# kaiwenShen/Do-You-Really-Need-to-Pay-2-20-Hedge-Fund-Strategy-Replication-via-Machine-Learning

Hardware: AMD Instinct MI355X
Metric: seq/sec/node MTSS-WGAN-GP train (24x32 windows) at 1/2/4/8 GPUs; W-dist parity (higher is better)
Workload: dtype fp32; 1 GPU; global_batch=262144, batch_per_gpu=262144, seq_len=24, features=32, parallelism=dp1

## Files before the change

do-you-really-need-to-pay-2-20-hedge-fund-strategy-replication-via-machine-learning_amd/csrc/bindings.cpp:

```cpp
#include <torch/extension.h>
#include <torch/library.h>
#include <ATen/hip/impl/HIPGuardImplMasqueradingAsCUDA.h>
#include <ATen/hip/impl/HIPStreamMasqueradingAsCUDA.h>

#include "kernels.h"
#include "poison.h"

#include <atomic>
#include <cmath>
#include <cstdlib>
#include <cstring>

std::atomic<bool>& hfrep::poison_flag() {
  static std::atomic<bool> f{[] {
    const char* e = getenv("HFREP_POISON");
    return e && e[0] == '1';
  }()};
  return f;
}

namespace {

using at::Tensor;
using c10::optional;
// ... 210 lines not shown
                                         (int)act, cur_stream(zx));
  TORCH_CHECK(ok, "lstm_fwd: hidden size ", H, " not instantiated (supported: 100, 64, 32)");
  return {hs, gates, cs};
}

Tensor lstm_bwd(Tensor dH, Tensor gates, Tensor cs, Tensor U, int64_t act) {
  CHECK_GPU(dH); CHECK_GPU(gates); CHECK_GPU(cs); same_dt(dH, gates); same_dt(dH, cs);
  const int B = gates.size(0), Tn = gates.size(1), H = gates.size(2) / 4;
  TORCH_CHECK(dH.sizes() == cs.sizes() && cs.size(2) == H, "lstm_bwd: shapes");
  check_lstm_U(U, H);
  GUARD(dH);
  Tensor dZ = out_empty_like(gates);
  const bool ok = hfrep::launch_lstm_bwd(dt_of(dH), dH.data_ptr(), gates.data_ptr(), cs.data_ptr(),
                                         U.data_ptr<float>(), dZ.data_ptr(), B, Tn, H, (int)act, cur_stream(dH));
  TORCH_CHECK(ok, "lstm_bwd: hidden size ", H, " not instantiated");
  return dZ;
}

std::tuple<Tensor, Tensor, Tensor> lstm_tfwd(Tensor dzx, Tensor gates, Tensor cs, Tensor U, int64_t act) {
  CHECK_GPU(dzx); CHECK_GPU(gates); CHECK_GPU(cs); same_dt(dzx, gates); same_dt(dzx, cs);
  TORCH_CHECK(dzx.sizes() == gates.sizes(), "lstm_tfwd: shapes");
  const int B = gates.size(0), Tn = gates.size(1), H = gates.size(2) / 4;
  check_lstm_U(U, H);
  GUARD(dzx);
  Tensor hds = out_empty({B, Tn, H}, dzx.options());
  Tensor zds = out_empty_like(gates);
  Tensor cds = out_empty({B, Tn, H}, dzx.options());
  const bool ok = hfrep::launch_lstm_tfwd(dt_of(dzx), dzx.data_ptr(), gates.data_ptr(), cs.data_ptr(),
                                          U.data_ptr<float>(), hds.data_ptr(), zds.data_ptr(), cds.data_ptr(), B, Tn,
                                          H, (int)act, cur_stream(dzx));
  TORCH_CHECK(ok, "lstm_tfwd: hidden size ", H, " not instantiated");
  return {hds, zds, cds};
}

std::tuple<Tensor, Tensor> lstm_tbwd(optional<Tensor> dH, Tensor dHd, Tensor gates, Tensor cs, Tensor zds, Tensor cds,
                                     Tensor U, int64_t act) {
  CHECK_GPU(dHd); CHECK_GPU(gates); CHECK_GPU(cs); CHECK_GPU(zds); CHECK_GPU(cds);
  same_dt(dHd, gates); same_dt(dHd, zds); same_dt(dHd, cds);
  if (dH.has_value()) { CHECK_GPU(*dH); same_dt(*dH, dHd); }
  const int B = gates.size(0), Tn = gates.size(1), H = gates.size(2) / 4;
  check_lstm_U(U, H);
  GUARD(dHd);
  Tensor dZ = out_empty_like(gates), dZd = out_empty_like(gates);
  const bool ok = hfrep::launch_lstm_tbwd(dt_of(dHd), ptr_or_null(dH), dHd.data_ptr(), gates.data_ptr(),
                                          cs.data_ptr(), zds.data_ptr(), cds.data_ptr(), U.data_ptr<float>(),
                                          dZ.data_ptr(), dZd.data_ptr(), B, Tn, H, (int)act, cur_stream(dHd));
  TORCH_CHECK(ok, "lstm_tbwd: hidden size ", H, " not instantiated");
  return {dZ, dZd};
}

bool lstmf_supported(int64_t H, int64_t K, int64_t act) { return hfrep::lstmf_supported((int)H, (int)K, (int)act); }
bool narrowf_supported(int64_t K, int64_t N) { return hfrep::narrowf_supported((int)K, (int)N); }
int64_t set_lstmf_fwd_impl(int64_t v) { return hfrep::set_lstmf_fwd_impl((int)v); }
int64_t set_lstmf_bwd_impl(int64_t v) { return hfrep::set_lstmf_bwd_impl((int)v); }

std::tuple<Tensor, Tensor> lstmf_fwd(Tensor x, Tensor W, optional<Tensor> b, Tensor U, int64_t act, bool save) {
  CHECK_F32(x); CHECK_F32(W);
  TORCH_CHECK(x.dim() == 3, "x must be (B, T, K)");
  const int B = x.size(0), Tn = x.size(1), K = x.size(2), H = U.size(0);
  check_lstm_U(U, H);
  TORCH_CHECK(W.size(0) == K && W.size(1) == 4 * H, "W must be (K, 4H)");
  if (b.has_value()) { CHECK_F32(*b); TORCH_CHECK(b->numel() == 4 * H, "bias size"); }
  TORCH_CHECK(hfrep::lstmf_supported(H, K, (int)act), "lstmf_fwd: unsupported H/K/act");
  GUARD(x);
  Tensor hs = out_empty({B, Tn, H}, x.options());
  Tensor tape = at::empty({save ? (int64_t)hfrep::lstmf_tape_elems(B, Tn) : 0}, x.options());
  const bool ok = hfrep::launch_lstmf_fwd(x.data_ptr<float>(), W.data_ptr<float>(),
                                          b.has_value() ? b->data_ptr<float>() : nullptr, U.data_ptr<float>(),
                                          hs.data_ptr<float>(), save ? tape.data_ptr<float>() : nullptr, B, Tn, K, H,
                                          (int)act, cur_stream(x));
  TORCH_CHECK(ok, "lstmf_fwd: launch failed");
  return {hs, tape};
}

std::tuple<Tensor, Tensor> lstmf_tfwd(Tensor xd, Tensor W, Tensor U, Tensor tape, int64_t act) {
  CHECK_F32(xd); CHECK_F32(W); CHECK_F32(tape);
  TORCH_CHECK(xd.dim() == 3, "xd must be (B, T, K)");
  const int B = xd.size(0), Tn = xd.size(1), K = xd.size(2), H = U.size(0);
  check_lstm_U(U, H);
  TORCH_CHECK(W.size(0) == K && W.size(1) == 4 * H, "W must be (K, 4H)");
  TORCH_CHECK(tape.numel() == (int64_t)hfrep::lstmf_tape_elems(B, Tn), "lstmf_tfwd: tape size");
  TORCH_CHECK(hfrep::lstmf_supported(H, K, (int)act), "lstmf_tfwd: unsupported H/K/act");
  GUARD(xd);
  Tensor hds = out_empty({B, Tn, H}, xd.options());
  Tensor ttape = at::empty_like(tape);
  const bool ok = hfrep::launch_lstmf_tfwd(xd.data_ptr<float>(), W.data_ptr<float>(), U.data_ptr<float>(),
                                           tape.data_ptr<float>(), hds.data_ptr<float>(), ttape.data_ptr<float>(), B, Tn,
                                           K, H, (int)act, cur_stream(xd));
  TORCH_CHECK(ok, "lstmf_tfwd: launch failed");
  return {hds, ttape};
}

static void check_head(const optional<Tensor>& d, const optional<Tensor>& w, const Tensor& like, int64_t B, int64_t n) {
  if (d.has_value()) {
    CHECK_F32(*d);
    TORCH_CHECK(d->numel() == B && d->device() == like.device(), "head adjoint factor: B fp32 values");
  }
  if (w.has_value()) {
    CHECK_F32(*w);
    TORCH_CHECK(w->numel() == n && w->device() == like.device(), "head weight: Tn H fp32 values");
  }
}

bool lstmf_ahd_supported() { return hfrep::lstmf_ahd_supported(); }

Tensor lstmf_bwd(optional<Tensor> dH, Tensor tape, Tensor U, int64_t act, int64_t B, int64_t Tn, optional<Tensor> hd,
// ... 629 lines not shown
  return (int64_t)reinterpret_cast<intptr_t>(hfrep::p2p_ipc_open(h, (int)device));
}

void p2p_close(int64_t ptr) { hfrep::p2p_ipc_close(reinterpret_cast<void*>((intptr_t)ptr)); }

void p2p_allreduce_(Tensor x, Tensor buf, std::vector<int64_t> peers, int64_t rank, int64_t cap, double scale,
                    double timeout_s) {
  CHECK_F32(x);
  TORCH_CHECK(buf.is_cuda() && buf.scalar_type() == at::kByte && buf.device() == x.device(),
              "p2p_allreduce_: buf must be this device's p2p_buffer");
  const int world = (int)peers.size();
  TORCH_CHECK(world >= 1 && world <= hfrep::kP2PMaxRanks && rank >= 0 && rank < world, "p2p_allreduce_: 1 <= world <= 8");
  TORCH_CHECK(x.numel() <= cap && buf.numel() >= (int64_t)hfrep::p2p_buffer_bytes(cap), "p2p_allreduce_: x exceeds cap");
  TORCH_CHECK(peers[rank] == (int64_t)reinterpret_cast<intptr_t>(buf.data_ptr()), "p2p_allreduce_: peers[rank] must be buf");
  hfrep::P2PPeers pp{};
  for (int r = 0; r < world; ++r) pp.base[r] = reinterpret_cast<char*>((intptr_t)peers[r]);
  TORCH_CHECK(timeout_s > 0, "p2p_allreduce_: timeout_s must be positive");
  GUARD(x);
  static thread_local int s_dev = -1;
  static thread_local double s_sec = -1;
  static thread_local uint64_t s_ticks = 0;
  if (s_dev != x.get_device() || s_sec != timeout_s) {
    s_ticks = hfrep::p2p_timeout_ticks(timeout_s, x.get_device());
    s_dev = x.get_device();
    s_sec = timeout_s;
  }
  hfrep::launch_p2p_allreduce(x.data_ptr<float>(), x.numel(), pp, (int)rank, world, cap, (float)scale, s_ticks,
                              cur_stream(x));
}

int64_t p2p_error(Tensor buf) {
  TORCH_CHECK(buf.is_cuda() && buf.scalar_type() == at::kByte, "p2p_error: a p2p_buffer tensor");
  GUARD(buf);
  return hfrep::p2p_read_error(buf.data_ptr());
}

}

TORCH_LIBRARY(hfrep, m) {
  m.def("linear(Tensor x, Tensor W, Tensor? b, int act, Tensor(a!)? out=None) -> Tensor");
  m.def("linear_dgrad(Tensor dz, Tensor W) -> Tensor");
  m.def("linear_wgrad_(Tensor x, Tensor dz, Tensor(a!) gW, Tensor(b!)? gb, int shiftT=0) -> ()");
  m.def("lstm_wgrad_(Tensor x, Tensor hs, Tensor dZ, Tensor(a!) gW, Tensor(b!) gU, Tensor(c!)? gb, Tensor? xd=None, Tensor? hds=None, Tensor? dZd=None, int impl=0) -> ()");
  m.def("act_fwd(Tensor x, int act) -> Tensor");
  m.def("act_bwd(Tensor dy, Tensor y, int act) -> Tensor");
  m.def("act_tangent_bwd(Tensor dyd, Tensor y, Tensor zd, int act) -> Tensor");
  m.def("lstm_fwd(Tensor zx, Tensor U, int act, bool save) -> (Tensor, Tensor, Tensor)");
  m.def("lstm_bwd(Tensor dH, Tensor gates, Tensor cs, Tensor U, int act) -> Tensor");
  m.def("lstm_tfwd(Tensor dzx, Tensor gates, Tensor cs, Tensor U, int act) -> (Tensor, Tensor, Tensor)");
  m.def("lstm_tbwd(Tensor? dH, Tensor dHd, Tensor gates, Tensor cs, Tensor zds, Tensor cds, Tensor U, int act) -> (Tensor, Tensor)");
  m.def("lstmf_supported(int H, int K, int act) -> bool", &lstmf_supported);
  m.def("narrowf_supported(int K, int N) -> bool", &narrowf_supported);
  m.def("set_lstmf_fwd_impl(int v) -> int", &set_lstmf_fwd_impl);
  m.def("set_lstmf_bwd_impl(int v) -> int", &set_lstmf_bwd_impl);
  m.def("lstmf_fwd(Tensor x, Tensor W, Tensor? b, Tensor U, int act, bool save) -> (Tensor, Tensor)");
  m.def("linear_head_cs(Tensor x, Tensor W, Tensor? b, int split, float wa, float wb, Tensor(a!) gW, Tensor(b!)? gb) -> Tensor");
  m.def("linear_head_cs_supported(int K) -> bool", &linear_head_cs_supported);
  m.def("lstmf_bwd(Tensor? dH, Tensor tape, Tensor U, int act, int B, int T, Tensor? hd=None, Tensor? hw=None, "
        "Tensor(a!)? ah_out=None) -> Tensor");
  m.def("lstmf_ahd_supported() -> bool", &lstmf_ahd_supported);
  m.def("lstmf_tbwd1(Tensor? dH, Tensor aH, Tensor tape, Tensor ttape, Tensor U, int act, int B, int T, Tensor? hd=None, "
        "Tensor? hw=None) -> Tensor");
  m.def("lstmf_tbwd(Tensor? dH, Tensor? dHd, Tensor tape, Tensor ttape, Tensor U, int act, int B, int T, Tensor? hd=None, "
        "Tensor? hdd=None, Tensor? hw=None) -> (Tensor, Tensor)");
  m.def("lstmf_tfwd(Tensor xd, Tensor W, Tensor U, Tensor tape, int act) -> (Tensor, Tensor)");
  m.def("lstmf_dgrad(Tensor dz, Tensor W, int impl=0) -> Tensor");
  m.def("lstm2_fwd(Tensor x, Tensor W, Tensor? b, Tensor U, int act, bool save) -> (Tensor, Tensor)");
  m.def("lstm2_bwd(Tensor? dH, Tensor tape, Tensor U, int act, Tensor? W=None, bool need_dz=True, Tensor? head_d=None, "
        "Tensor? head_w=None) -> (Tensor, Tensor)");
  m.def("lstm2_tfwd(Tensor xd, Tensor W, Tensor U, Tensor tape, int act) -> (Tensor, Tensor)");
  m.def("lstm2_tbwd(Tensor? dH, Tensor? dHd, Tensor tape, Tensor ttape, Tensor U, int act, Tensor? W=None, "
        "Tensor? head_d=None, Tensor? head_dd=None, Tensor? head_w=None) -> (Tensor, Tensor, Tensor, Tensor)");
  m.def("set_debug_poison(bool on) -> bool", &set_debug_poison);
  m.def("layernorm_fwd(Tensor x, Tensor gamma, Tensor beta, float eps, bool save=True, float pre_lrelu=-1.0) -> "
        "(Tensor, Tensor, Tensor)");
  m.def("layernorm_bwd_(Tensor dy, Tensor xhat, Tensor rstd, Tensor gamma, Tensor(a!)? ggamma, Tensor(b!)? gbeta) -> Tensor");
  m.def("layernorm_tfwd(Tensor xd, Tensor xhat, Tensor rstd, Tensor gamma) -> Tensor");
  m.def("layernorm_tbwd_(Tensor? dy, Tensor dyd, Tensor xd, Tensor xhat, Tensor rstd, Tensor gamma, "
        "Tensor(a!) ggamma, Tensor(b!) gbeta, bool need_dx) -> (Tensor, Tensor)");
  m.def("gp_coef(Tensor g, float weight) -> (Tensor, Tensor)");
  m.def("gp_coef_pack(Tensor g, float weight, Tensor w) -> (Tensor, Tensor)");
  m.def("gp_pack(Tensor pen, float weight, Tensor w) -> Tensor");
  m.def("gan_loss(Tensor p, int split, float la, float lb, int kind) -> (Tensor, Tensor)");
  m.def("im2col_causal(Tensor x, int k, int dil) -> Tensor");
  m.def("col2im_causal(Tensor dcols, int k, int dil, int C) -> Tensor");
  m.def("interpolate(Tensor real, Tensor fake, Tensor alpha) -> Tensor");
  m.def("philox_fill_(Tensor(a!) out, int seed, Tensor(b!) ctr, int dist) -> ()");
  m.def("sample_windows(Tensor data, int batch, int seed, Tensor(a!) ctr, ScalarType out_dtype, Tensor(b!)? dst=None) -> Tensor");
  m.def("ae_fit_supported(int A, int k, int batch) -> bool", &ae_fit_supported);
  m.def("ae_fit(Tensor[] Xt, Tensor[] Xv, Tensor[] order, Tensor(a!)[] We, Tensor(b!)[] Wd, Tensor(c!)[] mWe, "
        "Tensor(d!)[] vWe, Tensor(e!)[] mWd, Tensor(f!)[] vWd, Tensor(g!)[] step, Tensor(h!)[] m_cache, int[] patience, "
        "float lr, float b1, float b2, float eps, int batch, bool bf16) -> (Tensor, Tensor)");
  m.def("rmsprop_(Tensor(a!) p, Tensor g, Tensor(b!) ms, float lr, float rho, float eps, float clip, float gscale) -> ()");
  m.def("adam_(Tensor(a!) p, Tensor g, Tensor(b!) m, Tensor(c!) v, Tensor step, float lr, float b1, float b2, float eps, float clip, float gscale) -> ()");
  m.def("nadam_(Tensor(a!) p, Tensor g, Tensor(b!) m, Tensor(c!) v, Tensor step, Tensor m_cache, float lr, float b1, float b2, float eps, float gscale) -> ()");
  m.def("step_advance_(Tensor(a!) step, Tensor(b!)? m_cache, float b1) -> ()");
  m.def("clip_(Tensor(a!) p, float c) -> ()");
  m.def("wdist_sorted(Tensor x, Tensor ref_sorted) -> Tensor");
  m.def("ks_stat(Tensor x, Tensor ref_sorted) -> Tensor");
  m.def("acf_mean(Tensor x, int nlags) -> Tensor");
  m.def("nb_divergences(Tensor real, Tensor fake, Tensor theta, Tensor var, Tensor log_prior) -> Tensor");
  m.def("lp_cols(Tensor a, Tensor b) -> Tensor");
  m.def("p2p_buffer(int cap, int device) -> Tensor", &p2p_buffer);
  m.def("p2p_handle(Tensor buf) -> int[]");
  m.def("p2p_open(int[] handle, int device) -> int", &p2p_open);
  m.def("p2p_close(int ptr) -> ()", &p2p_close);
// ... 56 lines not shown
```

do-you-really-need-to-pay-2-20-hedge-fund-strategy-replication-via-machine-learning_amd/csrc/kernels.h:

```cpp
#pragma once
#include <hip/hip_runtime.h>
#include <stdint.h>

namespace hfrep {

enum DType : int { DT_F32 = 0, DT_BF16 = 1 };

bool launch_lstm_fwd(int dt, const void* zx, const float* U, void* hs, void* gates, void* cs, int B, int Tn, int H,
                     int act, hipStream_t s);
bool launch_lstm_bwd(int dt, const void* dH, const void* gates, const void* cs, const float* U, void* dZ, int B,
                     int Tn, int H, int act, hipStream_t s);
bool launch_lstm_tfwd(int dt, const void* dzx, const void* gates, const void* cs, const float* U, void* hds,
                      void* zds, void* cds, int B, int Tn, int H, int act, hipStream_t s);
bool launch_lstm_tbwd(int dt, const void* dH, const void* dHd, const void* gates, const void* cs, const void* zds,
                      const void* cds, const float* U, void* dZ, void* dZd, int B, int Tn, int H, int act,
                      hipStream_t s);

size_t lstm2_tape_elems(int B, int Tn);
bool lstm2_supported(int H, int K);
void launch_lstm2_fwd(const void* x, const float* W, const float* b, const float* U, void* hs, void* tape, int B, int Tn,
                      int K, int H, int act, hipStream_t s);
void launch_lstm2_tfwd(const void* xd, const float* W, const float* U, const void* tape, void* hds, void* ttape, int B,
                       int Tn, int K, int H, int act, hipStream_t s);
void launch_lstm2_bwd(const void* dH, const void* tape, const float* U, void* dZ, const float* W, void* dX, int K,
                      int B, int Tn, int H, int act, hipStream_t s, const void* head_d = nullptr,
                      const float* hw = nullptr);
void launch_lstm2_tbwd(const void* dH, const void* dHd, const void* tape, const void* ttape, const float* U, void* dZ,
                       void* dZd, const float* W, void* dX, void* dXd, int K, int B, int Tn, int H, int act,
                       hipStream_t s, const void* head_d = nullptr, const void* head_dd = nullptr,
                       const float* hw = nullptr);

bool lstmf_supported(int H, int K, int act);
size_t lstmf_tape_elems(int B, int Tn);
bool launch_lstmf_fwd(const float* x, const float* W, const float* b, const float* U, float* hs, float* tape, int B,
                      int Tn, int K, int H, int act, hipStream_t s);
bool launch_lstmf_tfwd(const float* xd, const float* W, const float* U, const float* tape, float* hds, float* ttape,
                       int B, int Tn, int K, int H, int act, hipStream_t s);
bool launch_lstmf_bwd(const float* dH, const float* tape, const float* U, float* dZ, int B, int Tn, int H, int act,
                      hipStream_t s, const float* hd = nullptr, const float* hw = nullptr, float* aH = nullptr);
bool lstmf_head_supported();
bool lstmf_ahd_supported();
bool launch_lstmf_tbwd1(const float* dH, const float* aH, const float* tape, const float* ttape, const float* U, float* dZ,
                        int B, int Tn, int H, int act, hipStream_t s, const float* hd = nullptr,
                        const float* hw = nullptr);
bool launch_lstmf_tbwd(const float* dH, const float* dHd, const float* tape, const float* ttape, const float* U, float* dZ,
                       float* dZd, int B, int Tn, int H, int act, hipStream_t s, const float* hd = nullptr,
                       const float* hdd = nullptr, const float* hw = nullptr);
int set_lstmf_fwd_impl(int v);
int set_lstmf_bwd_impl(int v);

bool lstmf_wgrad_supported(int K, int H, int N);
size_t lstmf_wgrad_workspace_floats(int M, int K, int impl = 0);
bool launch_lstmf_wgrad(const float* X, const float* Hs, const float* D, const float* Xd, const float* Hds, const float* Dd,
                        float* gW, float* gU, float* gb, int M, int K, int Tn, float* ws, hipStream_t s, int impl = 0);
bool lstmf_dgrad_supported(int N, int KO);
bool launch_lstmf_dgrad(const float* D, const float* W, float* X, int M, int N, int KO, hipStream_t s, int impl = 0);

bool ae_fit_supported(int A, int k, int batch);
struct AeFitJob {
  const float* Xt;
  const float* Xv;
  const int* order;
  float *We, *Wd, *mWe, *vWe, *mWd, *vWd, *step, *m_cache;
  double* hist;
  int* nep;
  int nt, nv, epochs, patience, k, pad_;
};
void launch_ae_fit(bool bf16, const AeFitJob* jobs, int njobs, int batch, float lr, float b1, float b2, float eps, int A,
                   hipStream_t s);

void launch_linear(int dt, const void* A, const float* W, const float* bias, void* C, int M, int N, int K,
                   int w_trans, int act, hipStream_t s);
bool fp32_exact_mode();
size_t wgrad_workspace_floats(int M, int K, int N);
void launch_wgrad(int dt, const void* X, const void* D, float* gW, float* gb, int M, int K, int N, int shiftT,
                  float* ws, hipStream_t s);

size_t lstm_wgrad2_workspace_floats(int M, int K, int Hd, int N);
void launch_lstm_wgrad2(const void* X0, const void* H0, const void* D0, const void* X1, const void* H1, const void* D1,
                        float* gW, float* gU, float* gb, int M, int K, int Hd, int N, int Tn, float* ws, hipStream_t s);
void launch_lstm_wgrad2_reduce(const float* ws, float* gW, float* gU, float* gb, int splits, int K, int Hd, int N,
                               hipStream_t s, int Ks = 0);
void launch_linear2(const void* A, const float* W, const float* bias, void* C, int M, int N, int K, int w_trans, int act,
                    hipStream_t s);

bool lstm_wgrad3_supported(int M, int K, int Hd, int N);
size_t lstm_wgrad3_workspace_floats(int K, int Hd, int N);
bool launch_lstm_wgrad3(const void* X0, const void* H0, const void* D0, const void* X1, const void* H1, const void* D1,
                        float* gW, float* gU, float* gb, int M, int K, int Hd, int N, int Tn, float* ws, hipStream_t s);

bool skinny_supported(int K, int N);
bool narrow_supported(int K, int N);
void launch_narrow_fwd(const void* x, const float* W, const float* b, void* y, int M, int K, int N, int act,
                       hipStream_t s);
bool narrowf_supported(int K, int N);
bool widef_supported(int K, int N);
void launch_widef(const float* x, const float* B, int sk, int sn, const float* b, float* y, int M, int K, int N,
                  int act, hipStream_t s);
void launch_narrowf(const float* x, const float* B, int sk, int sn, const float* b, float* y, int M, int K, int N,
                    int act, hipStream_t s);
void launch_skinny_fwd(int dt, const void* x, const float* W, const float* b, void* y, int M, int K, int N, int act,
// ... 84 lines not shown
```

do-you-really-need-to-pay-2-20-hedge-fund-strategy-replication-via-machine-learning_amd/csrc/lstm_f32.hip:

```cpp
#include "lstmf_dev.h"

#include <atomic>
#include <cstdlib>
#include <type_traits>
#include <stdexcept>

namespace hfrep {

namespace {

__device__ __forceinline__ rsrc_t ftile_rsrc(const float* base, int row0, int B, int Tn, int W) {
  row0 = __builtin_amdgcn_readfirstlane(row0);
  const int nr = base ? max(0, min(32, B - row0)) : 0;
  return make_rsrc(base + (nr ? (size_t)row0 * Tn * W : 0), nr * Tn * W * 4);
}

template <int K>
struct FGeo {
  static_assert(K >= 1 && K <= 112, "fp32 LSTM: K <= 112");
  static constexpr int KS = (K + 3) / 4;
  static constexpr int KQ = KS <= 12 ? 12 : 28;
  static constexpr int LR = KS <= 12 ? 56 : 120;
  static constexpr int NJ = (KS + 3) / 4;
};
// ... 1212 lines not shown
                cdn = f2_rnd(y[0] * gdot) + __builtin_fmaf(idot, y[2], __builtin_fmaf(fdot, cprev[i][n], y[1] * cst[i][n]));
              } else {
                cdn = __builtin_fmaf(y[0], gdot, f2_rnd(idot * y[2]) + (f2_rnd(y[1] * cst[i][n]) + f2_rnd(fdot * cprev[i][n])));
              }
              hd = f2_rnd(odot * ca) + f2_rnd(yd * cdn);
            } else {
              cdn = __builtin_fmaf(y[0], gdot, __builtin_fmaf(idot, y[2], __builtin_fmaf(y[1], cst[i][n], fdot * cprev[i][n])));
              hd = __builtin_fmaf(odot, ca, yd * cdn);
            }
            cst[i][n] = cdn;
            cprev[i][n] = c;
            hv = hd;
            hr = hv - __builtin_bit_cast(float, trunc_hi(hv));
            st4(f32x4{zd[0], zd[1], zd[2], zd[3]}, rt, tg);
            st1(cdn, rt, tc, 0);
          }
          {
            const int row = 16 * m + 4 * g + q;
            if (t0 + n < 24) {
              const uint32_t h1 = trunc_hi(hv);
              const uint32_t m1 = trunc_hi(hr);
              const uint32_t l1 = __builtin_bit_cast(uint32_t, hr - __builtin_bit_cast(float, m1));
              lds_char* dp = hnext + (row * FS_HR + ub + 4 * n) * 2;
              *reinterpret_cast<__attribute__((address_space(3))) uint16_t*>(dp) = (uint16_t)(h1 >> 16);
              *reinterpret_cast<__attribute__((address_space(3))) uint16_t*>(dp + FS_HPL) = (uint16_t)(m1 >> 16);
              *reinterpret_cast<__attribute__((address_space(3))) uint16_t*>(dp + 2 * FS_HPL) = (uint16_t)(l1 >> 16);
            } else {
              *reinterpret_cast<__attribute__((address_space(3))) float*>(hnext + 3 * FS_HPL + (row * 4 + j4) * 4) = hv;
            }
          }
          st1(hv, rh, v1, 0);
        }
      }
      xp.to_lds(xb + ((t + 1) & 1) * 32 * GX::LR, trash);
      lds_barrier();
    }
  }
}

template <int ACT, int KX, bool TAPE, bool TAN, int SKEW>
__global__ void __launch_bounds__(512, 1)
lstmf_fwds2_kernel(const float* __restrict__ x, const float* __restrict__ W, const float* __restrict__ bias,
                   const float* __restrict__ U, const float* __restrict__ ptape, float* __restrict__ hs,
                   float* __restrict__ tape, int B, int Tn) {
  static_assert(FGeo<KX>::KS <= 12, "split forward: K <= 48");
  extern __shared__ __attribute__((aligned(16))) float fsm[];
  constexpr bool PRIO = SKEW & 1, FLIP = SKEW & 2;
  const int v = __builtin_amdgcn_readfirstlane(threadIdx.x >> 6);
  if (v == 0) fwds2_run<ACT, KX, TAPE, TAN, 4, false, FLIP>(x, W, bias, U, ptape, hs, tape, B, Tn, fsm, v);
  else if (!PRIO || v < 4) fwds2_run<ACT, KX, TAPE, TAN, 3, false, FLIP>(x, W, bias, U, ptape, hs, tape, B, Tn, fsm, v);
  else fwds2_run<ACT, KX, TAPE, TAN, 3, true, FLIP>(x, W, bias, U, ptape, hs, tape, B, Tn, fsm, v);
}

constexpr int BS_LZ = 432;
constexpr int BS_PL = 32 * BS_LZ * 2;

template <int ACT, bool HEAD = false, bool AHD = false>
__global__ void __launch_bounds__(256, 1)
lstmf_bwds_kernel(const float* __restrict__ dH, const float* __restrict__ tape, const float* __restrict__ U,
                  float* __restrict__ dZ, int B, int Tn, const float* __restrict__ hd, const float* __restrict__ hw,
                  float* __restrict__ aH) {
  extern __shared__ __attribute__((aligned(16))) float fsm[];
  float* zt = fsm;
  float* ht = zt + 32 * BZ_LR;
  float* trash = ht + 32 * BH_LR;
  lds_char* trashp = (lds_char*)(trash + 4 * BZ_KQ);
  lds_char* zp = (lds_char*)(trash + 4 * BZ_KQ + 4);
  const int tid = threadIdx.x, lane = tid & 63;
  const int w = __builtin_amdgcn_readfirstlane(tid >> 6);
  const int q = lane & 3, g = lane >> 4, j4 = (lane & 15) >> 2, c16 = lane & 15;
  const int nrb = (B + 31) / 32;
  bf16x8 up[2][DS_KS][3];
#pragma unroll
  for (int e = 0; e < 2; ++e) {
    const int col = 16 * (2 * w + e) + c16;
    const bool ok = col < FH;
#pragma unroll
    for (int ks = 0; ks < DS_KS; ++ks) {
      f32x4 v[2];
#pragma unroll
      for (int j = 0; j < 8; ++j) {
        const int k = min(32 * ks + 8 * g + j, FG - 1);
        const float x = U[(ok ? col : 0) * FG + (k & 3) * FH + (k >> 2)];
        v[j >> 2][j & 3] = (ok && 32 * ks + 8 * g + j < FG) ? x : 0.f;
      }
      uint32_t p0[3][2], p1[3][2];
      split3(v[0], p0);
      split3(v[1], p1);
#pragma unroll
      for (int p = 0; p < 3; ++p) {
        up[e][ks][p] = __builtin_bit_cast(bf16x8, make_uint4(p0[p][0], p0[p][1], p1[p][0], p1[p][1]));
        if (e == 1 || ks < 8) asm volatile("" : "+a"(up[e][ks][p]));
      }
    }
  }
  const int ub = FUW * w + j4;
  const int hr = (4 * g + q) * BH_LR + ub, zw = (4 * g + q) * BZ_LR + ub;
  const int zpw = ((4 * g + q) * BS_LZ + 4 * ub) * 2;
  const int ao = (c16 * BS_LZ + 8 * g) * 2;
  const RevStore st(tid, Tn);
  const int tl = ftape_lane(w, lane), tcl = ftape_cell(w, lane);
  for (int rb = blockIdx.x; rb < nrb; rb += gridDim.x) {
    const int row0 = rb * 32;
    const rsrc_t rdh = ftile_rsrc(dH, row0, B, Tn, FH), rt = ftape_rsrc(tape, rb, nrb, Tn);
    const rsrc_t rz = ftile_rsrc(dZ, row0, B, Tn, FG);
    const rsrc_t rah = ftile_rsrc(AHD ? aH : nullptr, row0, B, Tn, FH);
// ... 66 lines not shown
#pragma unroll
      for (int ks = 0; ks < DS_KS; ++ks) {
        if (ks + 1 < DS_KS) {
#pragma unroll
          for (int p = 0; p < 3; ++p)
            af[(ks + 1) & 1][p] = *reinterpret_cast<const __attribute__((address_space(3))) bf16x8*>(ar + p * BS_PL + 64 * (ks + 1));
        }
        const bf16x8(&a)[3] = af[ks & 1];
#pragma unroll
        for (int e = 0; e < 2; ++e) acc[e] = mma_split6(a, up[e][ks], acc[e]);
        if (ks < FNT) cell(std::integral_constant<int, 1 - MA>{}, ks, hv[ks], t);
      }
#pragma unroll
      for (int ks = 0; ks < DS_KS; ++ks) {
        __builtin_amdgcn_sched_group_barrier(0x100, 3, 0);
#pragma unroll
        for (int i = 0; i < 12; ++i) {
          __builtin_amdgcn_sched_group_barrier(0x008, 1, 0);
          __builtin_amdgcn_sched_group_barrier(0x002, 3, 0);
        }
      }
      __builtin_amdgcn_sched_barrier(0);
#pragma unroll
      for (int e = 0; e < 2; ++e) {
        const bool ok = 2 * w + e < 7;
        float* hd = ok ? ht + (16 * MA + 4 * g) * BH_LR + 16 * (2 * w + e) + c16 : trash;
        const int hs = ok ? BH_LR : 0;
#pragma unroll
        for (int i = 0; i < 4; ++i) hd[i * hs] = acc[e][i];
      }
      lds_barrier();
    };
    for (int t = T1; t >= 0; --t) {
      phase(I1{}, t);
      phase(I0{}, t);
    }
    st.half<1, false>(zt, rz, Tn, 0, nr);
    __syncthreads();
  }
}

namespace {
template <int KX>
constexpr size_t fwdf_smem() {
  return (size_t)(2 * 32 * FGeo<KX>::LR + 2 * 32 * FGeo<FH>::LR + f_nwl<KX>() * 4 * FNT * 64 + 4) * 4;
}
static_assert(fwdf_smem<100>() <= F_LDS_MAX, "fp32 forward LDS");

template <int KX>
constexpr size_t fwds_smem() {
  return (size_t)(2 * 32 * FGeo<KX>::LR) * 4 + 2 * FS_HB + 16;
}
static_assert(fwds2_smem<32>() <= F_LDS_MAX, "two-wave split forward LDS");
static std::atomic<int>& fwdf_impl() {
  static std::atomic<int> v{fp32_exact() ? 1 : 3};
  return v;
}
static int fwdf_version() { return fwdf_impl().load(std::memory_order_relaxed); }
template <int ACT, int KX, bool TAPE, bool TAN, int SKEW>
void fwds2_launch(const float* x, const float* W, const float* b, const float* U, const float* pt, float* hs, float* tp,
                  int B, int Tn, hipStream_t s) {
  const int nrb = (B + 31) / 32, cus = device_cu_count();
  auto k = lstmf_fwds2_kernel<ACT, KX, TAPE, TAN, SKEW>;
  allow_lds(reinterpret_cast<const void*>(k));
  hipLaunchKernelGGL(k, dim3(nrb < cus ? nrb : cus), dim3(512), fwds2_smem<KX>(), s, x, W, b, U, pt, hs, tp, B, Tn);
}
template <int ACT, int KX, bool TAPE, bool TAN>
void fwdf_launch(const float* x, const float* W, const float* b, const float* U, const float* pt, float* hs, float* tp,
                 int B, int Tn, hipStream_t s) {
  const int nrb = (B + 31) / 32, cus = device_cu_count();
  if constexpr (KX == 32) {
    const int ver = fwdf_version();
    if (ver == 3) return fwds2_launch<ACT, KX, TAPE, TAN, HFREP_FWDS2_SKEW>(x, W, b, U, pt, hs, tp, B, Tn, s);
#ifdef HFREP_FWDS2_AB
    if constexpr (ACT == ACT_TANH) {
      if (ver == 30) return fwds2_launch<ACT, KX, TAPE, TAN, 0>(x, W, b, U, pt, hs, tp, B, Tn, s);
      if (ver == 31) return fwds2_launch<ACT, KX, TAPE, TAN, 1>(x, W, b, U, pt, hs, tp, B, Tn, s);
      if (ver == 32) return fwds2_launch<ACT, KX, TAPE, TAN, 2>(x, W, b, U, pt, hs, tp, B, Tn, s);
      if (ver == 33) return fwds2_launch<ACT, KX, TAPE, TAN, 3>(x, W, b, U, pt, hs, tp, B, Tn, s);
    }
#endif
  }
  if constexpr (FGeo<KX>::KS <= 8 || (FGeo<KX>::KS <= 12 && !TAN)) {
    if (fwdf_version() >= 2) {
      auto k = lstmf_fwds_kernel<ACT, KX, TAPE, TAN>;
      allow_lds(reinterpret_cast<const void*>(k));
      hipLaunchKernelGGL(k, dim3(nrb < cus ? nrb : cus), dim3(256), fwds_smem<KX>(), s, x, W, b, U, pt, hs, tp, B, Tn);
      return;
    }
  }
  auto k = lstmf_fwd_kernel<ACT, KX, TAPE, TAN>;
  allow_lds(reinterpret_cast<const void*>(k));
  hipLaunchKernelGGL(k, dim3(nrb < cus ? nrb : cus), dim3(256), fwdf_smem<KX>(), s, x, W, b, U, pt, hs, tp, B, Tn);
}
template <int KX, bool TAPE, bool TAN>
void fwdf_act(int act, const float* x, const float* W, const float* b, const float* U, const float* pt, float* hs,
              float* tp, int B, int Tn, hipStream_t s) {
  switch (act) {
    case ACT_LINEAR: fwdf_launch<ACT_LINEAR, KX, TAPE, TAN>(x, W, b, U, pt, hs, tp, B, Tn, s); break;
    case ACT_SIGMOID: fwdf_launch<ACT_SIGMOID, KX, TAPE, TAN>(x, W, b, U, pt, hs, tp, B, Tn, s); break;
    default: fwdf_launch<ACT_TANH, KX, TAPE, TAN>(x, W, b, U, pt, hs, tp, B, Tn, s); break;
  }
}
template <bool TAPE, bool TAN>
bool fwdf_k(int K, int act, const float* x, const float* W, const float* b, const float* U, const float* pt, float* hs,
            float* tp, int B, int Tn, hipStream_t s) {
  switch (K) {
    case 32: fwdf_act<32, TAPE, TAN>(act, x, W, b, U, pt, hs, tp, B, Tn, s); return true;
    case 35: fwdf_act<35, TAPE, TAN>(act, x, W, b, U, pt, hs, tp, B, Tn, s); return true;
    case 36: fwdf_act<36, TAPE, TAN>(act, x, W, b, U, pt, hs, tp, B, Tn, s); return true;
    case 100: fwdf_act<100, TAPE, TAN>(act, x, W, b, U, pt, hs, tp, B, Tn, s); return true;
    default: return false;
  }
}
}

int set_lstmf_fwd_impl(int v) { return fwdf_impl().exchange(v); }

bool lstmf_supported(int H, int K, int act) {
  return H == FH && (K == 32 || K == 35 || K == 36 || K == 100) && (act == ACT_LINEAR || act == ACT_SIGMOID || act == ACT_TANH);
}

bool launch_lstmf_fwd(const float* x, const float* W, const float* b, const float* U, float* hs, float* tape, int B,
                      int Tn, int K, int H, int act, hipStream_t s) {
  if (!lstmf_supported(H, K, act) || B <= 0 || Tn <= 0) return false;
  if (tape) return fwdf_k<true, false>(K, act, x, W, b, U, nullptr, hs, tape, B, Tn, s);
  return fwdf_k<false, false>(K, act, x, W, b, U, nullptr, hs, nullptr, B, Tn, s);
}

bool launch_lstmf_tfwd(const float* xd, const float* W, const float* U, const float* tape, float* hds, float* ttape,
                       int B, int Tn, int K, int H, int act, hipStream_t s) {
  if (!lstmf_supported(H, K, act) || B <= 0 || Tn <= 0) return false;
  return fwdf_k<true, true>(K, act, xd, W, nullptr, U, tape, hds, ttape, B, Tn, s);
}

static std::atomic<int>& bwdf_impl() {
  static std::atomic<int> v{fp32_exact() ? 2 : 3};
  return v;
}
template <int ACT>
void bwdf_launch(const float* dH, const float* tape, const float* U, float* dZ, int B, int Tn, hipStream_t s,
                 const float* hd, const float* hw, float* aH) {
  const int ver = bwdf_impl().load(std::memory_order_relaxed);
  const int nrb = (B + 31) / 32, cus = device_cu_count();
  const size_t sm = (size_t)(32 * BZ_LR + 32 * BH_LR + 4 * BZ_KQ) * 4;
  if (ver != 2) {
    auto go = [&](auto k) {
      allow_lds(reinterpret_cast<const void*>(k));
      hipLaunchKernelGGL(k, dim3(nrb < cus ? nrb : cus), dim3(256), sm + 16 + 3 * BS_PL, s, dH, tape, U, dZ, B, Tn, hd,
                         hw, aH);
    };
    if (aH) {
      if (hd) go(lstmf_bwds_kernel<ACT, true, true>);
      else go(lstmf_bwds_kernel<ACT, false, true>);
    } else {
      if (hd) go(lstmf_bwds_kernel<ACT, true>);
      else go(lstmf_bwds_kernel<ACT, false>);
    }
    return;
  }
  if (aH) throw std::runtime_error("lstmf_bwd: the exact-fp32 BPTT does not store the h adjoints (lstmf_ahd_supported)");
  if (hd) throw std::runtime_error("lstmf_bwd: the exact-fp32 BPTT takes a materialised dH (lstmf_head_supported)");
  auto k = lstmf_bwdp_kernel<ACT>;
  allow_lds(reinterpret_cast<const void*>(k));
  hipLaunchKernelGGL(k, dim3(nrb < cus ? nrb : cus), dim3(512), sm, s, dH, tape, U, dZ, B, Tn);
}
static_assert((32 * BZ_LR + 32 * BH_LR + 4 * BZ_KQ) * 4 + 16 + 3 * BS_PL <= F_LDS_MAX, "split BPTT LDS");
int set_lstmf_bwd_impl(int v) { return bwdf_impl().exchange(v); }
bool lstmf_head_supported() { return bwdf_impl().load(std::memory_order_relaxed) != 2; }
bool lstmf_ahd_supported() { return bwdf_impl().load(std::memory_order_relaxed) != 2; }
// ... 63 lines not shown
```

Before: 1.580 million seq/s.

## Add eight-wave fused LSTM forward kernel for the K=100 layer

New measurement: 1.613 million seq/s, median of 6. +2.1%, better.

```diff
diff --git a/do-you-really-need-to-pay-2-20-hedge-fund-strategy-replication-via-machine-learning_amd/csrc/bindings.cpp b/do-you-really-need-to-pay-2-20-hedge-fund-strategy-replication-via-machine-learning_amd/csrc/bindings.cpp
--- a/do-you-really-need-to-pay-2-20-hedge-fund-strategy-replication-via-machine-learning_amd/csrc/bindings.cpp
+++ b/do-you-really-need-to-pay-2-20-hedge-fund-strategy-replication-via-machine-learning_amd/csrc/bindings.cpp
@@ -286,6 +286,7 @@
 bool lstmf_supported(int64_t H, int64_t K, int64_t act) { return hfrep::lstmf_supported((int)H, (int)K, (int)act); }
 bool narrowf_supported(int64_t K, int64_t N) { return hfrep::narrowf_supported((int)K, (int)N); }
 int64_t set_lstmf_fwd_impl(int64_t v) { return hfrep::set_lstmf_fwd_impl((int)v); }
+int64_t set_lstmf_fwd100_impl(int64_t v) { return hfrep::set_lstmf_fwd100_impl((int)v); }
 int64_t set_lstmf_bwd_impl(int64_t v) { return hfrep::set_lstmf_bwd_impl((int)v); }
 
 std::tuple<Tensor, Tensor> lstmf_fwd(Tensor x, Tensor W, optional<Tensor> b, Tensor U, int64_t act, bool save) {
@@ -1021,6 +1022,7 @@
   m.def("lstmf_supported(int H, int K, int act) -> bool", &lstmf_supported);
   m.def("narrowf_supported(int K, int N) -> bool", &narrowf_supported);
   m.def("set_lstmf_fwd_impl(int v) -> int", &set_lstmf_fwd_impl);
+  m.def("set_lstmf_fwd100_impl(int v) -> int", &set_lstmf_fwd100_impl);
   m.def("set_lstmf_bwd_impl(int v) -> int", &set_lstmf_bwd_impl);
   m.def("lstmf_fwd(Tensor x, Tensor W, Tensor? b, Tensor U, int act, bool save) -> (Tensor, Tensor)");
   m.def("linear_head_cs(Tensor x, Tensor W, Tensor? b, int split, float wa, float wb, Tensor(a!) gW, Tensor(b!)? gb) -> Tensor");
diff --git a/do-you-really-need-to-pay-2-20-hedge-fund-strategy-replication-via-machine-learning_amd/csrc/kernels.h b/do-you-really-need-to-pay-2-20-hedge-fund-strategy-replication-via-machine-learning_amd/csrc/kernels.h
--- a/do-you-really-need-to-pay-2-20-hedge-fund-strategy-replication-via-machine-learning_amd/csrc/kernels.h
+++ b/do-you-really-need-to-pay-2-20-hedge-fund-strategy-replication-via-machine-learning_amd/csrc/kernels.h
@@ -47,6 +47,7 @@
                        float* dZd, int B, int Tn, int H, int act, hipStream_t s, const float* hd = nullptr,
                        const float* hdd = nullptr, const float* hw = nullptr);
 int set_lstmf_fwd_impl(int v);
+int set_lstmf_fwd100_impl(int v);
 int set_lstmf_bwd_impl(int v);
 
 bool lstmf_wgrad_supported(int K, int H, int N);
diff --git a/do-you-really-need-to-pay-2-20-hedge-fund-strategy-replication-via-machine-learning_amd/csrc/lstm_f32.hip b/do-you-really-need-to-pay-2-20-hedge-fund-strategy-replication-via-machine-learning_amd/csrc/lstm_f32.hip
--- a/do-you-really-need-to-pay-2-20-hedge-fund-strategy-replication-via-machine-learning_amd/csrc/lstm_f32.hip
+++ b/do-you-really-need-to-pay-2-20-hedge-fund-strategy-replication-via-machine-learning_amd/csrc/lstm_f32.hip
@@ -1288,6 +1288,230 @@
   else fwds2_run<ACT, KX, TAPE, TAN, 3, true, FLIP>(x, W, bias, U, ptape, hs, tape, B, Tn, fsm, v);
 }
 
+constexpr int F2_NWR3 = 13, F2_NWR4 = 5;
+constexpr int F2_G3 = (25 - F2_NWR3) / 4, F2_G4 = (25 - F2_NWR4) / 4;
+static_assert(F2_NWR3 + 4 * F2_G3 == 25 && F2_NWR4 + 4 * F2_G4 == 25, "W^T k-steps in LDS come in fours");
+__device__ __forceinline__ constexpr int f2_woff(int gt) { return gt < 4 ? F2_G4 * gt : F2_G3 * gt + (F2_G4 - F2_G3) * 4; }
+constexpr size_t fwd2_smem() {
+  return (size_t)(2 * 32 * (FGeo<100>::LR + FGeo<FH>::LR) + 4) * 4 + (size_t)(F2_G3 * 25 + (F2_G4 - F2_G3) * 4) * 1024;
+}
+
+template <int ACT, bool TAPE, bool TAN, int NT>
+__device__ __forceinline__ void fwd2_run(const float* __restrict__ x, const float* __restrict__ W,
+                                         const float* __restrict__ bias, const float* __restrict__ U,
+                                         const float* __restrict__ ptape, float* __restrict__ hs,
+                                         float* __restrict__ tape, int B, int Tn, float* fsm, int v) {
+  constexpr int KX = 100;
+  using GX = FGeo<KX>;
+  using GH = FGeo<FH>;
+  constexpr bool BIG = NT == 4;
+  constexpr int NWR = BIG ? F2_NWR4 : F2_NWR3, NG = BIG ? F2_G4 : F2_G3;
+  static_assert(GX::KS == 25 && GH::KS == 25 && (NT == 3 || NT == 4), "tile plan of the K = 100 layer");
+  float* xb = fsm;
+  float* hb = xb + 2 * 32 * GX::LR;
+  float* trash = hb + 2 * 32 * GH::LR;
+  f32x4* wl = (f32x4*)(trash + 4);
+  const int tid = threadIdx.x, lane = tid & 63;
+  const int q = lane & 3, g = lane >> 4, j4 = (lane & 15) >> 2;
+  const int t0 = v ? 3 * v + 1 : 0;
+  const int nrb = (B + 31) / 32;
+
+  for (int i = tid; i < 2 * 32 * (GX::LR + GH::LR); i += 512) fsm[i] = 0.f;
+
+  constexpr float GSC = ACT == ACT_TANH ? -2.f * kLog2e : ACT == ACT_SIGMOID ? -kLog2e : 1.f;
+  const float sc = TAN ? 1.f : (q == 2 ? GSC : -kLog2e);
+  float uf[GH::KS][NT], wf[NWR][NT], bq[NT];
+  int tsl[NT];
+#pragma unroll
+  for (int n = 0; n < NT; ++n) {
+    const int gt = t0 + n;
+    const int cl = q * FH + 4 * gt + j4;
+    tsl[n] = ftape_lane(gt / FNT, 0) + ((gt % FNT) * FT_SLOT) * 4;
+#pragma unroll
+    for (int ks = 0; ks < GH::KS; ++ks) {
+      uf[ks][n] = U[(4 * ks + g) * FG + cl] * sc;
+      asm volatile("" : "+v"(uf[ks][n]));
+    }
+#pragma unroll
+    for (int ks = 0; ks < NWR; ++ks) {
+      wf[ks][n] = W[(4 * ks + g) * FG + cl] * sc;
+      asm volatile("" : "+v"(wf[ks][n]));
+    }
+#pragma unroll
+    for (int gi = 0; gi < NG; ++gi) {
+      f32x4 wv;
+#pragma unroll
+      for (int s4 = 0; s4 < 4; ++s4) wv[s4] = W[(4 * (NWR + 4 * gi + s4) + g) * FG + cl] * sc;
+      wl[(f2_woff(gt) + gi) * 64 + lane] = wv;
+    }
+    const float bv = bias ? bias[cl] : 0.f;
+    bq[n] = !TAN ? f2_rnd(bv * sc) : 0.f;
+  }
+  const bool glin = !TAN && ACT == ACT_LINEAR && q == 2;
+  const float am = q == 2 ? 2.f : 1.f, bm = q == 2 ? -1.f : 0.f;
+  const int ax = (lane & 15) * GX::LR + g * GX::KQ, ah = (lane & 15) * GH::LR + g * GH::KQ;
+  const int hw = (4 * g + q) * GH::LR + j4 * GH::KQ + t0;
+  const f32x4* wlw = wl + f2_woff(t0) * 64 + lane;
+  FXPart<KX> xp;
+  const bool xld = v >= 4;
+  __syncthreads();
+
+  for (int rb = blockIdx.x; rb < nrb; rb += gridDim.x) {
+    const int row0 = rb * 32;
+    const rsrc_t rx = ftile_rsrc(x, row0, B, Tn, KX);
+    const rsrc_t rh = ftile_rsrc(hs, row0, B, Tn, FH);
+    const rsrc_t rt = ftape_rsrc(TAPE ? tape : nullptr, rb, nrb, Tn);
+    const rsrc_t rp = ftape_rsrc(TAN ? ptape : nullptr, rb, nrb, Tn);
+    const int vp0 = ((4 * g + q) * Tn * FH + 4 * t0 + j4) * 4;
+    float cprev[TAN ? 2 : 1][NT];
+    if constexpr (TAN) {
+#pragma unroll
+      for (int m = 0; m < 2; ++m)
+#pragma unroll
+        for (int n = 0; n < NT; ++n) cprev[m][n] = 0.f;
+    }
+    float cst[2][NT];
+#pragma unroll
+    for (int m = 0; m < 2; ++m)
+#pragma unroll
+      for (int n = 0; n < NT; ++n) cst[m][n] = 0.f;
+    if constexpr (!BIG) {
+      xp.set(Tn, tid & 255);
+      if (!xld) {
+#pragma unroll
+        for (int j = 0; j < FXPart<KX>::NJ; ++j) { xp.goff[j] = kOOB; xp.lpos[j] = -1; }
+      }
+      xp.load(rx, Tn, 0, true);
+    }
+    for (int i = tid; i < 32 * GH::LR; i += 512) hb[i] = 0.f;
+    if constexpr (!BIG) xp.to_lds(xb, trash);
+    __syncthreads();
+    for (int t = 0; t < Tn; ++t) {
+      const float* xcur = xb + (t & 1) * 32 * GX::LR;
+      const float* hcur = hb + (t & 1) * 32 * GH::LR;
+      float* hnext = hb + ((t + 1) & 1) * 32 * GH::LR;
+      if constexpr (!BIG) xp.load(rx, Tn, t + 1, t + 1 < Tn);
+#pragma unroll
+      for (int m = 0; m < 2; ++m) {
+        f32x4 pg[TAN ? NT : 1];
+        float pc[TAN ? NT : 1];
+        const int p1 = vp0 + (16 * m * Tn + t) * FH * 4;
+        const int tb = t * FT_STEP * 4 + ftape_slot(m, 0);
+        if constexpr (TAN) {
+#pragma unroll
+          for (int n = 0; n < NT; ++n) {
+            pg[n] = ld4(rp, lane * 16 + (tb + tsl[n]));
+            pc[n] = ld1(rp, (256 + lane) * 4 + (tb + tsl[n]), 0);
+          }
+        }
+        f32x4 acc[NT];
+#pragma unroll
+        for (int n = 0; n < NT; ++n) acc[n] = f32x4{0.f, 0.f, 0.f, 0.f};
+        f32x4 w4[NT];
+#pragma unroll
+        for (int j = 0; j < GX::NJ; ++j) {
+          const f32x4 a4 = *reinterpret_cast<const f32x4*>(xcur + ax + 16 * m * GX::LR + 4 * j);
+#pragma unroll
+          for (int s = 0; s < 4; ++s) {
+            const int ks = 4 * j + s;
+            if (ks >= GX::KS) break;
+            if (ks >= NWR && (ks - NWR) % 4 == 0) {
+#pragma unroll
+              for (int n = 0; n < NT; ++n) w4[n] = wlw[(n * NG + (ks - NWR) / 4) * 64];
+            }
+#pragma unroll
+            for (int n = 0; n < NT; ++n) {
+              const float bw = ks < NWR ? wf[ks < NWR ? ks : 0][n] : w4[n][(ks >= NWR ? ks - NWR : 0) & 3];
+              acc[n] = mma4(a4[s], bw, acc[n]);
+            }
+          }
+          __builtin_amdgcn_sched_barrier(0);
+        }
+#pragma unroll
+        for (int j = 0; j < GH::NJ; ++j) {
+          const f32x4 a4 = *reinterpret_cast<const f32x4*>(hcur + ah + 16 * m * GH::LR + 4 * j);
+#pragma unroll
+          for (int s = 0; s < 4; ++s) {
+            const int ks = 4 * j + s;
+            if (ks >= GH::KS) break;
+#pragma unroll
+            for (int n = 0; n < NT; ++n) acc[n] = mma4(a4[s], uf[ks][n], acc[n]);
+          }
+          __builtin_amdgcn_sched_barrier(0);
+        }
+#pragma unroll
+        for (int n = 0; n < NT; ++n) {
+          const int v1 = p1 + 16 * n;
+          const int tg = lane * 16 + (tb + tsl[n]), tc = (256 + lane) * 4 + (tb + tsl[n]);
+          const f32x4 zs = acc[n];
+          float hv;
+          if constexpr (!TAN) {
+            float y[4];
+#pragma unroll
+            for (int e4 = 0; e4 < 4; ++e4) {
+              const float s_ = zs[e4] + bq[n];
+              const float r_ = __builtin_amdgcn_rcpf(1.f + __builtin_amdgcn_exp2f(s_));
+              float e = r_;
+              if constexpr (ACT == ACT_TANH) e = __builtin_fmaf(am, r_, bm);
+              y[e4] = glin ? s_ : e;
+            }
+            quad_transpose(y, q);
+            const float cn = __builtin_fmaf(y[1], cst[m][n], y[0] * y[2]);
+            float ca;
+            if constexpr (ACT == ACT_TANH) ca = __builtin_fmaf(__builtin_amdgcn_rcpf(1.f + __builtin_amdgcn_exp2f(GSC * cn)), 2.f, -1.f);
+            else if constexpr (ACT == ACT_SIGMOID) ca = __builtin_amdgcn_rcpf(1.f + __builtin_amdgcn_exp2f(GSC * cn));
+            else ca = cn;
+            hv = y[3] * ca;
+            cst[m][n] = cn;
+            if constexpr (TAPE) {
+              st4(f32x4{y[0], y[1], y[2], y[3]}, rt, tg);
+              st1(cn, rt, tc, 0);
+            }
+          } else {
+            float zd[4] = {zs[0], zs[1], zs[2], zs[3]};
+            quad_transpose(zd, q);
+            const f32x4 y = pg[n];
+            const float idot = y[0] * (1.f - y[0]) * zd[0], fdot = y[1] * (1.f - y[1]) * zd[1];
+            const float dg = ACT == ACT_TANH ? __builtin_fmaf(-y[2], y[2], 1.f) : ACT == ACT_SIGMOID ? y[2] * (1.f - y[2]) : 1.f;
+            const float gdot = dg * zd[2], odot = y[3] * (1.f - y[3]) * zd[3];
+            const float c = pc[n];
+            const float ca = act_f(ACT, c);
+            const float dc = ACT == ACT_TANH ? __builtin_fmaf(-ca, ca, 1.f) : ACT == ACT_SIGMOID ? ca * (1.f - ca) : 1.f;
+            const float yd = y[3] * dc;
+            const float fc = __builtin_fmaf(fdot, cprev[m][n], y[1] * cst[m][n]);
+            float cdn = __builtin_fmaf(y[0], gdot, __builtin_fmaf(idot, y[2], fc));
+            if (m == 0 && (t0 + n) % FNT == 4) {
+              if constexpr (ACT == ACT_LINEAR) cdn = f2_rnd(y[0] * gdot) + (f2_rnd(idot * y[2]) + (f2_rnd(fdot * cprev[m][n]) + f2_rnd(y[1] * cst[m][n])));
+              else cdn = __builtin_fmaf(y[0], gdot, f2_rnd(idot * y[2]) + fc);
+            }
+            hv = __builtin_fmaf(odot, ca, yd * cdn);
+            cst[m][n] = cdn;
+            cprev[m][n] = c;
+            st4(f32x4{zd[0], zd[1], zd[2], zd[3]}, rt, tg);
+            st1(cdn, rt, tc, 0);
+          }
+          hnext[hw + 16 * m * GH::LR + n] = hv;
+          st1(hv, rh, v1, 0);
+        }
+      }
+      if constexpr (!BIG) xp.to_lds(xb + ((t + 1) & 1) * 32 * GX::LR, trash);
+      lds_barrier();
+    }
+  }
+}
+
+template <int ACT, int KX, bool TAPE, bool TAN>
+__global__ void __launch_bounds__(512, 1)
+lstmf_fwd2_kernel(const float* __restrict__ x, const float* __restrict__ W, const float* __restrict__ bias,
+                  const float* __restrict__ U, const float* __restrict__ ptape, float* __restrict__ hs,
+                  float* __restrict__ tape, int B, int Tn) {
+  static_assert(KX == 100, "the eight-wave exact forward is the K = 100 layer's");
+  extern __shared__ __attribute__((aligned(16))) float fsm[];
+  const int v = __builtin_amdgcn_readfirstlane(threadIdx.x >> 6);
+  if (v == 0) fwd2_run<ACT, TAPE, TAN, 4>(x, W, bias, U, ptape, hs, tape, B, Tn, fsm, v);
+  else fwd2_run<ACT, TAPE, TAN, 3>(x, W, bias, U, ptape, hs, tape, B, Tn, fsm, v);
+}
+
 constexpr int BS_LZ = 432;
 constexpr int BS_PL = 32 * BS_LZ * 2;
 
@@ -1460,11 +1684,24 @@
   return (size_t)(2 * 32 * FGeo<KX>::LR) * 4 + 2 * FS_HB + 16;
 }
 static_assert(fwds2_smem<32>() <= F_LDS_MAX, "two-wave split forward LDS");
+static_assert(fwd2_smem() <= F_LDS_MAX, "eight-wave exact forward LDS");
 static std::atomic<int>& fwdf_impl() {
   static std::atomic<int> v{fp32_exact() ? 1 : 3};
   return v;
 }
 static int fwdf_version() { return fwdf_impl().load(std::memory_order_relaxed); }
+static std::atomic<int>& fwdf100_impl() {
+  static std::atomic<int> v{2};
+  return v;
+}
+template <int ACT, int KX, bool TAPE, bool TAN>
+void fwd2_launch(const float* x, const float* W, const float* b, const float* U, const float* pt, float* hs, float* tp,
+                 int B, int Tn, hipStream_t s) {
+  const int nrb = (B + 31) / 32, cus = device_cu_count();
+  auto k = lstmf_fwd2_kernel<ACT, KX, TAPE, TAN>;
+  allow_lds(reinterpret_cast<const void*>(k));
+  hipLaunchKernelGGL(k, dim3(nrb < cus ? nrb : cus), dim3(512), fwd2_smem(), s, x, W, b, U, pt, hs, tp, B, Tn);
+}
 template <int ACT, int KX, bool TAPE, bool TAN, int SKEW>
 void fwds2_launch(const float* x, const float* W, const float* b, const float* U, const float* pt, float* hs, float* tp,
                   int B, int Tn, hipStream_t s) {
@@ -1477,6 +1714,10 @@
 void fwdf_launch(const float* x, const float* W, const float* b, const float* U, const float* pt, float* hs, float* tp,
                  int B, int Tn, hipStream_t s) {
   const int nrb = (B + 31) / 32, cus = device_cu_count();
+  if constexpr (KX == 100) {
+    if (fwdf100_impl().load(std::memory_order_relaxed) == 2)
+      return fwd2_launch<ACT, KX, TAPE, TAN>(x, W, b, U, pt, hs, tp, B, Tn, s);
+  }
   if constexpr (KX == 32) {
     const int ver = fwdf_version();
     if (ver == 3) return fwds2_launch<ACT, KX, TAPE, TAN, HFREP_FWDS2_SKEW>(x, W, b, U, pt, hs, tp, B, Tn, s);
@@ -1524,6 +1765,7 @@
 }
 
 int set_lstmf_fwd_impl(int v) { return fwdf_impl().exchange(v); }
+int set_lstmf_fwd100_impl(int v) { return fwdf100_impl().exchange(v); }
 
 bool lstmf_supported(int H, int K, int act) {
   return H == FH && (K == 32 || K == 35 || K == 36 || K == 100) && (act == ACT_LINEAR || act == ACT_SIGMOID || act == ACT_TANH);
```
